# lgautier/fastq-and-furious

Hardware: AMD Instinct MI355X
Metric: GB/s FASTQ parsed (higher is better)
Workload: dtype u8; 1 GPU; single-1g; description=S-single 150 bp synthetic FASTQ, 1073741522 bytes/GPU, 3334601 records/GPU, diagnostic=False, bytes_per_gpu=1073741522, records_per_gpu=3334601, total_bytes=1073741522, total_records=3334601

## Files before the change

### fastq-and-furious_amd/csrc/ffq_rows4.h

```cpp
#pragma once
#include "ffq_chain.h"

namespace ffq {

constexpr int SB_TILES = 64;
constexpr int R4_LIST = SLOT + 8;

struct Fast4Hdr {
    long long j0;
    int32_t attempt;
    int32_t dense_seen;
    unsigned long long irr_min;
    unsigned long long term_min;
    long long n_lines;
};

struct TermInfo4 {
    int64_t pos[6];
    int32_t status;
    int32_t final_;
};

struct TileQ {
    long long kfirst;
    int32_t nrec;
    uint32_t qsum;
};

__device__ __forceinline__ long long tile_ordinal_base(const LineIndex &L, const long long *sbbase, int t, int lane)
{
    const int sb = t / SB_TILES, t0 = sb * SB_TILES;
    const uint32_t c = (t0 + lane < t) ? L.cnt[t0 + lane] : 0u;
    return sbbase[sb] + (long long)wave_sum_u32(c) + L.s;
}

__global__ __launch_bounds__(256) void k_sum64(const uint32_t *__restrict__ src, int stride, int64_t nsrc,
                                               unsigned int *__restrict__ dst, int ndst)
{
    const int b = blockIdx.x * 4 + __builtin_amdgcn_readfirstlane((int)(threadIdx.x >> 6)), lane = threadIdx.x & 63;
    if (b >= ndst) return;
    const int64_t i = (int64_t)b * 64 + lane;
    const uint32_t v = (i < nsrc) ? src[i * stride] : 0u;
    const uint32_t t = wave_sum_u32(v);
    if (lane == 0) dst[b] = t;
}

__global__ __launch_bounds__(1024) void k_sbscan(LineIndex L, int nsb, long long *__restrict__ sbbase, int64_t offset,
                                                 Fast4Hdr *hdr, const unsigned int *__restrict__ presum)
{
    __shared__ long long s_w[16];
    __shared__ uint32_t s_sum[16][64];
    const int tid = threadIdx.x, lane = tid & 63, wid = tid >> 6;
    if (wid == 15) {
        const int tq = (int)min((int64_t)max(L.ntiles - 1, 0), max((int64_t)0, (offset - L.s) >> TILE_SHIFT));
        uint32_t sink = (L.n > 0) ? (uint32_t)L.d[0] : 0u;
        if (L.ntiles > 0) sink += L.cnt[tq] + L.ent[(int64_t)tq * SLOT + lane * 4];
        if (tq + 1 < L.ntiles) sink += L.cnt[tq + 1] + L.ent[(int64_t)(tq + 1) * SLOT + (lane & 15) * 4];
        asm volatile("" ::"v"(sink));
    }
    long long carry = 0;
    if (presum) {
        for (int c0 = 0; c0 < nsb; c0 += 16 * 1024) {
            uint32_t pv[16];
#pragma unroll
            for (int k = 0; k < 16; k++) {
                const int b = c0 + k * 1024 + tid;
                pv[k] = (b < nsb) ? presum[b] : 0u;
            }
#pragma unroll
            for (int k = 0; k < 16; k++) {
                const int b = c0 + k * 1024 + tid;
                if (c0 + k * 1024 >= nsb) continue;
                const uint32_t v = pv[k];
                const uint32_t incl = wave_incl_scan(v);
                if (lane == 63) s_w[wid] = (long long)incl;
                __syncthreads();
                long long wpre = 0, tot = 0;
#pragma unroll
                for (int q = 0; q < 16; q++) {
                    const long long t = s_w[q];
                    if (q < wid) wpre += t;
                    tot += t;
                }
                if (b < nsb) sbbase[b] = carry + wpre + (long long)(incl - v);
                __syncthreads();
                carry += tot;
            }
        }
    } else
    for (int b0 = 0; b0 < nsb; b0 += 1024) {
        const int b = b0 + tid;
        uint32_t part[16];
        const int64_t tw0 = ((int64_t)(b0 + wid * 64) << 6) + lane * 4;
        if (tw0 + (15 << 8) + 4 <= L.ntiles - (63 - lane) * 4) {
            uint4 x[16];
#pragma unroll
            for (int j = 0; j < 16; j++) x[j] = *reinterpret_cast<const uint4 *>(L.cnt + tw0 + ((int64_t)j << 8));
#pragma unroll
            for (int j = 0; j < 16; j++) part[j] = x[j].x + x[j].y + x[j].z + x[j].w;
        } else {
#pragma unroll
            for (int j = 0; j < 16; j++) {
                const int64_t t = tw0 + ((int64_t)j << 8);
                uint32_t a = 0;
                for (int q = 0; q < 4; q++)
                    if (t + q < L.ntiles) a += L.cnt[t + q];
                part[j] = a;
            }
        }
#pragma unroll
        for (int j = 0; j < 16; j++) {
            uint32_t r = part[j];
            r += (uint32_t)__builtin_amdgcn_update_dpp(0, (int)r, 0x111, 0xf, 0xf, false);
            r += (uint32_t)__builtin_amdgcn_update_dpp(0, (int)r, 0x112, 0xf, 0xf, false);
            r += (uint32_t)__builtin_amdgcn_update_dpp(0, (int)r, 0x114, 0xf, 0xf, false);
            r += (uint32_t)__builtin_amdgcn_update_dpp(0, (int)r, 0x118, 0xf, 0xf, false);
            if ((lane & 15) == 15) s_sum[wid][4 * j + (lane >> 4)] = r;
        }
        __syncthreads();
        const uint32_t v = (b < nsb) ? s_sum[wid][lane] : 0u;
        const uint32_t incl = wave_incl_scan(v);
        if (lane == 63) s_w[wid] = (long long)incl;
        __syncthreads();
        long long wpre = 0, tot = 0;
#pragma unroll
        for (int q = 0; q < 16; q++) {
            const long long t = s_w[q];
            if (q < wid) wpre += t;
            tot += t;
        }
        if (b < nsb) sbbase[b] = carry + wpre + (long long)(incl - v);
        __syncthreads();
        carry += tot;
    }
    __syncthreads();
    if (tid == 0) {
        hdr->n_lines = carry;
        hdr->irr_min = ~0ull;
        hdr->term_min = ~0ull;
        hdr->attempt = 1;
        hdr->dense_seen = 0;
        hdr->j0 = -1;
        const GAcc a(L);
        H h = a.before();
        long long ord = -1;
        long long found = -1;
        int64_t P; int fl;
        int tskip = (int)min((int64_t)L.ntiles, max((int64_t)0, (offset - L.s) >> TILE_SHIFT));
        if (tskip > 0) {
            long long o = sbbase[tskip / SB_TILES] + L.s;
            for (int t = (tskip / SB_TILES) * SB_TILES; t < tskip; t++) o += L.cnt[t];
            h = H{tskip - 1, 0x7FFFFFF0};
            ord = o - 1;
        }
        bool gave_up = false;
        for (int steps = 0;; steps++) {
            if (steps > 4096) { gave_up = true; break; }
            bool ok;
            if (h.tile >= 0 && h.i == 0x7FFFFFF0) {
                int t = h.tile + 1;
                while (t < L.ntiles && L.cnt[t] == 0) t++;
                ok = t < L.ntiles;
                if (ok) { h.tile = t; h.i = 0; }
            } else ok = a.next(h);
            if (!ok) break;
            ord++;
            a.get(h, P, fl);
            if ((fl & FL_AT) && P >= offset) { found = ord; break; }
        }
        if (gave_up) hdr->attempt = 0;
        else {
            hdr->j0 = found;
            if (found >= 0) {
                H h2 = h;
                if (a.next(h2) && a.next(h2)) {
                    a.get(h2, P, fl);
                    if (!(fl & FL_PLUS)) hdr->attempt = 0;
                }
            }
        }
    }
}

constexpr uint8_t FZ_ALL = 0xFE;
template <int FUSED, bool DENSE>
__global__ __launch_bounds__(256, DENSE ? 4 : 8) void k_rows4(LineIndex L, const long long *__restrict__ sbbase, int eof,
                                               int64_t add, Fast4Hdr *hdr, TermInfo4 *__restrict__ tinfo,
                                               int64_t *__restrict__ table, int64_t table_cap,
                                               uint32_t *__restrict__ qrel, TileQ *__restrict__ tileq,
                                               int64_t *__restrict__ p4s, int64_t p4_cap,
                                               int64_t fz_stride, const uint8_t *__restrict__ fz_phase,
                                               int64_t *__restrict__ fz_qoff)
{
    __shared__ __attribute__((aligned(16))) uint16_t s_ent_all[4][R4_LIST];
    __shared__ uint32_t s_la_all[4][8];
    __shared__ __attribute__((aligned(16))) int32_t s_rows_all[4][64 * 6];
    const int wid = __builtin_amdgcn_readfirstlane((int)(threadIdx.x >> 6)), lane = threadIdx.x & 63;
    const int t = blockIdx.x * 4 + wid;
    if (t >= L.ntiles) return;
    const int attempt = hdr->attempt;
    const long long j0 = hdr->j0;
    const unsigned long long irr0 = hdr->irr_min;
    const unsigned long long term0 = hdr->term_min;
    uint16_t *s_ent = s_ent_all[wid];
    uint32_t *s_la = s_la_all[wid];
    int32_t *s_rows = s_rows_all[wid];
    const int64_t len = L.len();

    const int tn = min(t + 1, L.ntiles - 1);
    const int sb = t / SB_TILES, t0 = sb * SB_TILES;
    const uint16_t *src = L.ent + (int64_t)t * SLOT;
    const uint32_t c_raw = L.cnt[t];
    const uint2 v0 = *reinterpret_cast<const uint2 *>(src + 4 * lane);
    const uint32_t c1_raw = L.cnt[tn];
    const uint2 vla_raw = *reinterpret_cast<const uint2 *>(L.ent + (int64_t)tn * SLOT + 4 * (lane & 1));
    const uint32_t cb_raw = L.cnt[min(t0 + lane, L.ntiles - 1)];
    const long long sbb = sbbase[sb];
    constexpr bool fused = FUSED != 0, in_place = FUSED == 2;
    uint32_t fzph = 0;
    if (fused) fzph = fz_phase[t];
    asm volatile("" ::"v"(c_raw), "v"(v0.x), "v"(v0.y), "v"(c1_raw), "v"(vla_raw.x), "v"(vla_raw.y), "v"(cb_raw),
                 "v"(sbb), "s"(attempt), "s"(j0), "v"(fzph));
    const int c = (int)c_raw;
    const bool have_next = t + 1 < L.ntiles;
    const int c1 = have_next ? (int)c1_raw : 0;
    const uint2 vla = vla_raw;
    const long long ob = sbb + (long long)wave_sum_u32((t0 + lane < t) ? cb_raw : 0u) + L.s;
    if (!attempt) return;
    if (ob - j0 > 0 && ((unsigned long long)((ob - j0) >> 2) > irr0 || (unsigned long long)((ob - j0) >> 2) > (term0 >> 24))) return;
    if (c > SLOT && (!DENSE || fused)) {
        if (lane == 0 && (hdr->irr_min != 0ull || !hdr->dense_seen)) { atomicMin(&hdr->irr_min, 0ull); hdr->dense_seen = 1; }
        return;
    }
    if (fused) {
        const uint32_t want = (uint32_t)(((j0 + 3 - ob) % 4 + 4) % 4);
        const bool wrong = in_place ? (fzph != (uint32_t)FZ_ALL && fzph != want) : (c > 0 && fzph != want);
        if ((wrong || j0 != 0) && lane == 0 && hdr->irr_min != 0ull) atomicMin(&hdr->irr_min, 0ull);
    }
    const int pre = (t == 0 && L.s) ? 1 : 0;
    if (c + pre == 0 && t != 0) return;
    const int64_t tbase = ((int64_t)t << TILE_SHIFT) + L.s;
    const int64_t tb_add = tbase + add;
    const int32_t lim = (int32_t)min(len - tbase, (int64_t)0x7FFFFFF0);
    if (j0 < 0) {
        if (t == 0 && lane == 0) {
            TermInfo4 &ti = tinfo[0];
            for (int i = 0; i < 6; i++) ti.pos[i] = -1;
            ti.status = ST_HEAD_BEG; ti.final_ = 0;
            atomicMin(&hdr->term_min, 0ull);
        }
        return;
    }
    const int ntot = pre + c;
    const int nch = DENSE ? (ntot + SLOT - 1) / SLOT : 1;
    const uint16_t *dsrc = nullptr;
    if (DENSE && c > SLOT) {
        const unsigned long long at = L.ovf[t] & OVF_MASK;
        if (at + (unsigned long long)c > L.pool_cap) {
            if (lane == 0) atomicMin(&hdr->irr_min, 0ull);
            return;
        }
        dsrc = L.pool + at;
    }
    long long kfirst = -1;
    int nrec_tile = 0;
    bool tile_term_done = false;
    uint32_t qrun = 0;
    for (int ch = 0; ch < nch; ch++) {
    const int e_lo = DENSE ? ch * SLOT : 0;
    const int nown = DENSE ? min(SLOT, ntot - e_lo) : ntot;
    const bool sent0 = pre && e_lo == 0;
    const long long obl = ob - pre + e_lo;
    if (DENSE && ch > 0) wave_sync();
    if (DENSE && dsrc) {
        for (int x0 = 8 * lane; x0 < nown; x0 += 512) {
            const int ph = e_lo + x0 - pre;
            if (ph >= 0 && ph + 8 <= c) {
                typedef uint32_t u32x4u __attribute__((ext_vector_type(4), aligned(2)));
                const u32x4u v = *reinterpret_cast<const u32x4u *>(dsrc + ph);
                *reinterpret_cast<uint4 *>(s_ent + x0) = make_uint4(v.x, v.y, v.z, v.w);
            } else {
#pragma unroll
                for (int q = 0; q < 8; q++)
                    if (ph + q >= 0 && ph + q < c) s_ent[x0 + q] = dsrc[ph + q];
            }
        }
    }
    if (sent0) {
        if (lane == 0) {
            const uint8_t b0 = L.n > 0 ? L.d[0] : 0;
            const uint32_t fl = (b0 == '@') ? FL_AT : (b0 == '+') ? FL_PLUS : 0;
            s_ent[0] = (uint16_t)(fl << 14);
        }
        if (!(DENSE && dsrc)) {
            const uint32_t x[4] = {v0.x & 0xFFFFu, v0.x >> 16, v0.y & 0xFFFFu, v0.y >> 16};
#pragma unroll
            for (int i = 0; i < 4; i++)
                if (4 * lane + i < c) s_ent[1 + 4 * lane + i] = (uint16_t)x[i];
        }
    } else if (!(DENSE && dsrc)) {
        *reinterpret_cast<uint2 *>(s_ent + 4 * lane) = v0;
    }
    if (!(DENSE && dsrc))
        for (int i = 256 + lane; i < c; i += 64) {
            s_ent[pre + i] = src[i];
        }
    int nl = nown;
    bool idx_end = false;
    const bool last_ch = !DENSE || ch == nch - 1;
    bool la_simple;
    int32_t la_add = TILE;
    if (last_ch) {
        la_simple = have_next && c1 >= 5 && (c1 <= SLOT || DENSE);
        if (la_simple && (!DENSE || c1 <= SLOT)) {
            if (lane < 2) {
                const uint32_t x[4] = {vla.x & 0xFFFFu, vla.x >> 16, vla.y & 0xFFFFu, vla.y >> 16};
#pragma unroll
                for (int i = 0; i < 4; i++)
                    if (4 * lane + i < 5) {
                        s_la[4 * lane + i] = ((1u << TILE_SHIFT) + (x[i] & OFF_MASK)) | ((x[i] >> 14) << 30);
                        s_ent[nl + 4 * lane + i] = (uint16_t)x[i];
                    }
            }
            nl += 5;
        } else if (la_simple) {
            const unsigned long long at1 = L.ovf[t + 1] & OVF_MASK;
            if (at1 + 5ull <= L.pool_cap) {
                if (lane < 5) {
                    const uint32_t e = L.pool[at1 + lane];
                    s_la[lane] = ((1u << TILE_SHIFT) + (e & OFF_MASK)) | ((e >> 14) << 30);
                    s_ent[nl + lane] = (uint16_t)e;
                }
                nl += 5;
            } else la_simple = false;
        }
    } else {
        la_simple = ntot - (e_lo + nown) >= 5;
        la_add = 0;
        if (la_simple) {
            if (lane < 5) {
                const uint32_t e = dsrc[e_lo + nown - pre + lane];
                s_la[lane] = (e & OFF_MASK) | ((e >> 14) << 30);
                s_ent[nl + lane] = (uint16_t)e;
            }
            nl += 5;
        }
    }
    if (!la_simple) {
        int tt = last_ch ? t + 1 : t, pp = last_ch ? 0 : e_lo + nown - pre, got = 0;
        while (got < 5) {
            if (tt >= L.ntiles) { idx_end = true; break; }
            const int cc = (tt == t) ? c : (int)L.cnt[tt];
            if (cc > SLOT && !DENSE) break;
            if (pp >= cc) { tt++; pp = 0; if (tt - t > 60000) break; continue; }
            const uint16_t *es = L.ent + (int64_t)tt * SLOT;
            if (cc > SLOT) {
                const unsigned long long at1 = L.ovf[tt] & OVF_MASK;
                if (at1 + (unsigned long long)cc > L.pool_cap) break;
                es = L.pool + at1;
            }
            const int take = min(cc - pp, 5 - got);
            if (lane < take) {
                const uint32_t e = es[pp + lane];
                s_la[got + lane] = (((uint32_t)(tt - t) << TILE_SHIFT) + (e & OFF_MASK)) | ((e >> 14) << 30);
            }
            got += take;
            pp += take;
        }
        nl += got;
    }
    wave_sync();

    long long kfirst_ch = -1;
    int nrec_ch = 0;
    {
        long long i0 = (obl >= j0) ? ((4 - ((obl - j0) & 3)) & 3) : (j0 - obl);
        if (i0 < nown) {
            kfirst_ch = (obl + i0 - j0) >> 2;
            nrec_ch = (int)((nown - i0 + 3) >> 2);
            if (kfirst < 0) kfirst = kfirst_ch;
        }
        for (int r0 = 0; r0 < nrec_ch; r0 += 64) {
            const int r = r0 + lane;
            const bool act = r < nrec_ch;
            const int i = (int)i0 + 4 * r;
            int cls = 0;
            bool fin = false;
            int32_t f0 = 0, f1 = 0, f3 = 0, f4 = 0, f5 = 0;
            bool usual = false;
            {
                const int ic = min(i, R4_LIST - 5);
                const uint32_t e0 = s_ent[ic], e1 = s_ent[ic + 1], e2 = s_ent[ic + 2], e3 = s_ent[ic + 3],
                               e4 = s_ent[ic + 4];
                const int32_t x0 = (sent0 && ic == 0) ? -1 : (int32_t)(e0 & OFF_MASK) + ((ic >= nown) ? la_add : 0);
                const int32_t x1 = (int32_t)(e1 & OFF_MASK) + ((ic + 1 >= nown) ? la_add : 0);
                const int32_t x2 = (int32_t)(e2 & OFF_MASK) + ((ic + 2 >= nown) ? la_add : 0);
                const int32_t x3 = (int32_t)(e3 & OFF_MASK) + ((ic + 3 >= nown) ? la_add : 0);
                const int32_t x4 = (int32_t)(e4 & OFF_MASK) + ((ic + 4 >= nown) ? la_add : 0);
                const int32_t qe = x3 + x2 - x1;
                usual = act & (i + 4 < nl) & (la_simple | (i + 4 < nown))
                      & (x1 <= lim - 2)
                      & (((e2 >> 14) & FL_PLUS) != 0) & (x2 >= x1 + 2)
                      & (x2 + 2 < lim) & (x3 <= lim - 2)
                      & !((x3 - x2 - 1 > 1) & (x3 - x2 != x1 - x0))
                      & (qe + 2 < lim)
                      & (((e4 >> 14) & FL_AT) != 0) & (x4 >= qe - 1);
                f0 = x0 + 1; f1 = x1; f3 = x2; f4 = x3 + 1; f5 = qe;
                if (fused && usual && x4 != qe) atomicMin(&hdr->irr_min, (unsigned long long)(kfirst_ch + r));
            }
            if (act && !usual) {
                int64_t p0 = 0, p1 = 0, p3 = 0, p4 = 0, p5 = 0;
                int status = ST_COMPLETE;
                const long long k = kfirst_ch + r;
                const int have = nl - i;
                auto POS = [&](int q) -> int64_t {
                    const int e = i + q;
                    if (e >= nown) return tbase + (int64_t)(s_la[e - nown] & 0x3FFFFFFFu);
                    if (sent0 && e == 0) return (int64_t)0;
                    return tbase + (int64_t)(s_ent[e] & OFF_MASK);
                };
                auto FLG = [&](int q) -> uint32_t {
                    const int e = i + q;
                    return (e >= nown) ? (s_la[e - nown] >> 30) : ((uint32_t)s_ent[e] >> 14);
                };
                const int64_t P0 = POS(0);
                p0 = P0 + 1; p1 = p3 = p4 = p5 = -1;
                if (have < 2) { cls = idx_end ? 2 : 1; status = ST_HEAD_END; }
                else {
                    const int64_t P1 = POS(1);
                    if (P1 > len - 2) { cls = 2; status = ST_HEAD_END; }
                    else {
                        p1 = P1;
                        if (have < 3) { cls = idx_end ? 2 : 1; status = ST_SEQ_END; }
                        else {
                            const int64_t P2 = POS(2);
                            if (!(FLG(2) & FL_PLUS) || P2 < P1 + 2) cls = 1;
                            else {
                                p3 = P2;
                                if (P2 + 2 >= len) { cls = 2; status = ST_QUALHEAD_END; }
                                else if (have < 4) { cls = idx_end ? 2 : 1; status = ST_QUALHEAD_END; }
                                else {
                                    const int64_t P3 = POS(3);
                                    if (P3 > len - 2) { cls = 2; status = ST_QUALHEAD_END; }
                                    else if ((P3 - P2 - 1 > 1) && (P3 - P2 != P1 - P0)) { cls = 2; status = ST_INVALID; }
                                    else {
                                        p4 = P3 + 1;
                                        const int64_t qe = p4 + P2 - P1 - 1;
                                        if (qe + 2 >= len) {
                                            cls = 2; status = ST_QUAL_END;
                                            if (eof && qe < len) { p5 = qe; fin = true; }
                                        } else {
                                            p5 = qe;
                                            if (have < 5) cls = idx_end ? 3 : 1;
                                            else if (!(FLG(4) & FL_AT) || POS(4) < qe - 1) cls = 1;
                                        }
                                    }
                                }
                            }
                        }
                    }
                }
                if (fused && (cls == 0 || cls == 3 || (cls == 2 && fin)) && !(have >= 5 && POS(4) == p5)) cls = 1;
                {
                    const unsigned long long im = __ballot(cls == 1);
                    if (cls == 1 && lane == __ffsll((long long)im) - 1 &&
                        (unsigned long long)k < __hip_atomic_load(&hdr->irr_min, __ATOMIC_RELAXED, __HIP_MEMORY_SCOPE_AGENT))
                        atomicMin(&hdr->irr_min, (unsigned long long)k);
                }
                if (cls == 2 || cls == 3) {
                    const unsigned long long kk = (unsigned long long)(cls == 3 ? k + 1 : k);
                    const unsigned long long mine = (kk << 24) | (unsigned long long)(t & 0xFFFFFF);
                    if (mine < __hip_atomic_load(&hdr->term_min, __ATOMIC_RELAXED, __HIP_MEMORY_SCOPE_AGENT)) atomicMin(&hdr->term_min, mine);
                }
                f0 = (int32_t)(p0 - tbase); f1 = (int32_t)(p1 - tbase); f3 = (int32_t)(p3 - tbase);
                f4 = (int32_t)(p4 - tbase); f5 = (int32_t)(p5 - tbase);
                const unsigned long long tm = __ballot(cls == 2 || cls == 3);
                if (tm != 0ull && !tile_term_done && lane == __ffsll((long long)tm) - 1) {
                    TermInfo4 ti;
                    if (cls == 3) {
                        for (int q = 0; q < 6; q++) ti.pos[q] = -1;
                        ti.status = ST_HEAD_BEG; ti.final_ = 0;
                    } else {
                        ti.pos[0] = p0; ti.pos[1] = p1; ti.pos[2] = (p1 >= 0) ? p1 + 1 : -1;
                        ti.pos[3] = p3; ti.pos[4] = p4; ti.pos[5] = p5;
                        ti.status = status; ti.final_ = fin ? 1 : 0;
                    }
                    tinfo[t] = ti;
                }
            }
            if (__ballot(act && (cls == 2 || cls == 3)) != 0ull) tile_term_done = true;
            const bool emit = act && (cls == 0 || cls == 3 || (cls == 2 && fin));
            if (in_place) {
                if (emit && kfirst_ch + r < p4_cap) fz_qoff[kfirst_ch + r] = ((long long)t << TILE_SHIFT) + f4;
            } else if (fused) {
                const uint32_t ql = emit ? (uint32_t)(f5 - f4) : 0u;
                const uint32_t incl = wave_incl_scan(ql);
                if (emit && kfirst_ch + r < p4_cap) {
                    const int32_t x3 = f4 - 1;
                    long long q = ((long long)t + (x3 >> TILE_SHIFT)) * fz_stride;
                    if (x3 < TILE) {
                        int32_t head = 0;
                        const int e0 = (int)i0 - pre;
                        if (kfirst_ch > 0 && e0 >= 1)
                            head = (int32_t)(s_ent[e0 + pre] & OFF_MASK) - (int32_t)(s_ent[e0 - 1 + pre] & OFF_MASK) - 1;
                        q += head + (long long)(qrun + incl - ql);
                    }
                    fz_qoff[kfirst_ch + r] = q;
                }
                qrun += (uint32_t)__shfl((int)incl, 63);
            } else if (qrel) {
                const uint32_t ql = emit ? (uint32_t)(f5 - f4) : 0u;
                const uint32_t incl = wave_incl_scan(ql);
                if (act && kfirst_ch + r < p4_cap) qrel[kfirst_ch + r] = qrun + incl - ql;
                if (emit && kfirst_ch + r < p4_cap) p4s[kfirst_ch + r] = tb_add + f4;
                qrun += (uint32_t)__shfl((int)incl, 63);
            }
            int2 *mine = reinterpret_cast<int2 *>(s_rows + lane * 6);
            mine[0] = make_int2(f0, f1); mine[1] = make_int2(f1 + 1, f3); mine[2] = make_int2(f4, f5);
            wave_sync();
            const unsigned long long em = __ballot(emit);
            const int64_t rowbase = kfirst_ch + r0;
            const int2 *srcr = reinterpret_cast<const int2 *>(s_rows);
            longlong2 *dst = reinterpret_cast<longlong2 *>(table + rowbase * 6);
#pragma unroll
            for (int u = 0; u < 3; u++) {
                const int q = lane + u * 64;
                const int row = q / 3;
                if (((em >> row) & 1ull) && rowbase + row < table_cap) {
                    typedef long long i64x2 __attribute__((ext_vector_type(2)));
                    const int2 vv = srcr[q];
                    i64x2 t; t.x = tb_add + vv.x; t.y = tb_add + vv.y;
                    __builtin_nontemporal_store(t, reinterpret_cast<i64x2 *>(dst + q));
                }
            }
            wave_sync();
        }
    }
    nrec_tile += nrec_ch;
    }
    if (qrel && lane == 0 && nrec_tile > 0) tileq[t] = TileQ{kfirst, nrec_tile, qrun};
}

__global__ __launch_bounds__(1024) void k_qscan4(const unsigned int *__restrict__ sbq, int nsb,
                                                 long long *__restrict__ sbqbase)
{
    __shared__ long long s_v[1024];
    const int tid = threadIdx.x;
    long long carry = 0;
    for (int b0 = 0; b0 < nsb; b0 += 1024) {
        const int b = b0 + tid;
        const long long v = (b < nsb) ? (long long)sbq[b] : 0;
        s_v[tid] = v;
        __syncthreads();
        for (int d = 1; d < 1024; d <<= 1) {
            long long x = 0;
            if (tid >= d) x = s_v[tid - d];
            __syncthreads();
            s_v[tid] += x;
            __syncthreads();
        }
        if (b < nsb) sbqbase[b] = carry + s_v[tid] - v;
        const long long tot = s_v[1023];
        __syncthreads();
        carry += tot;
    }
}

__global__ __launch_bounds__(256) void k_qfix4(int ntiles, const Fast4Hdr *__restrict__ hdr,
                                               const TileQ *__restrict__ tileq,
                                               const long long *__restrict__ sbqbase,
                                               const uint32_t *__restrict__ qrel, int64_t *__restrict__ qoff,
                                               int64_t table_cap, int64_t *__restrict__ qdir, int64_t qdir_cap)
{
    const int wid = __builtin_amdgcn_readfirstlane((int)(threadIdx.x >> 6)), lane = threadIdx.x & 63;
    const int t = (blockIdx.x * 4 + wid) * 2;
    if (t >= ntiles) return;
    const int attempt = hdr->attempt;
    const int t0 = (t / SB_TILES) * SB_TILES;
    const TileQ me0 = tileq[t];
    TileQ me1 = tileq[min(t + 1, ntiles - 1)];
    const uint32_t bq = tileq[min(t0 + lane, ntiles - 1)].qsum;
    const long long sbb = sbqbase[t / SB_TILES];
    asm volatile("" ::"v"(me0.kfirst), "v"(me0.nrec), "v"(me0.qsum), "v"(me1.kfirst), "v"(me1.nrec), "v"(me1.qsum),
                 "v"(bq), "v"(sbb), "s"(attempt));
    if (!attempt) return;
    if (t + 1 >= ntiles) me1.nrec = 0;
    const int64_t base0 = sbb + (int64_t)wave_sum_u32((t0 + lane < t) ? bq : 0u);
    const int64_t base1 = base0 + (int64_t)(me0.nrec > 0 ? me0.qsum : 0u);
    const int64_t i0 = me0.kfirst + lane, i1 = me1.kfirst + lane;
    const bool a0 = lane < me0.nrec && i0 < table_cap, a1 = lane < me1.nrec && i1 < table_cap;
    const int64_t l0 = a0 ? (int64_t)qrel[i0] : 0, l1 = a1 ? (int64_t)qrel[i1] : 0;
    asm volatile("" ::"v"(l0), "v"(l1));
    auto fix = [&](const TileQ &me, int64_t base, int r0, int64_t loc, bool act) {
        const int r = r0 + lane;
        const int64_t idx = me.kfirst + r;
        int64_t nxt = ((int64_t)__shfl((int)(loc >> 32), lane + 1) << 32) | (uint32_t)__shfl((int)(uint32_t)loc, lane + 1);
        if (r + 1 >= me.nrec) nxt = me.qsum;
        else if (lane == 63) nxt = (idx + 1 < table_cap) ? (int64_t)qrel[idx + 1] : (int64_t)me.qsum;
        if (act) {
            qoff[idx] = base + loc;
            qdir_mark(qdir, qdir_cap, base + loc, nxt - loc, idx);
        }
    };
    auto rest = [&](const TileQ &me, int64_t base) {
        for (int r0 = 64; r0 < me.nrec; r0 += 64) {
            const int64_t idx = me.kfirst + r0 + lane;
            const bool act = r0 + lane < me.nrec && idx < table_cap;
            fix(me, base, r0, act ? (int64_t)qrel[idx] : 0, act);
        }
    };
    if (me0.nrec > 0) fix(me0, base0, 0, l0, a0);
    if (me1.nrec > 0) fix(me1, base1, 0, l1, a1);
    if (me0.nrec > 64) rest(me0, base0);
    if (me1.nrec > 64) rest(me1, base1);
}

__global__ void k_qtotal4(DevRes *res, const int64_t *__restrict__ table, int64_t table_cap,
                          int64_t *__restrict__ qoff, Pub pb)
{
    if (threadIdx.x != 0 || blockIdx.x != 0) return;
    if (res->fallback) { publish(pb, res); return; }
    const int64_t n = res->n_records;
    int64_t tot = 0;
    if (n > 0 && n <= table_cap) tot = qoff[n - 1] + (table[(n - 1) * 6 + 5] - table[(n - 1) * 6 + 4]);
    res->n_qual_bytes = tot;
    if (n <= table_cap) qoff[n] = tot;
    publish(pb, res);
}

__global__ void k_finalize4(LineIndex L, Fast4Hdr *hdr, const TermInfo4 *__restrict__ tinfo, int eof,
                            int64_t offset, int64_t add, const int64_t *__restrict__ table, int64_t table_cap,
                            DevRes *res, Pub pb, const uint32_t *__restrict__ fz_bad = nullptr)
{
    if (threadIdx.x != 0 || blockIdx.x != 0) return;
    res->n_lines = hdr->n_lines;
    res->n_qual_bytes = 0;
    res->term_group = -1;
    res->has_final = 0;
    const unsigned long long tm = hdr->term_min, im = hdr->irr_min;
    const unsigned long long tk = tm >> 24;
    res->fused_bad = fz_bad ? (int32_t)*fz_bad : 0;
    res->fast4_dense = hdr->dense_seen;
    if (!hdr->attempt || tm == ~0ull || (im != ~0ull && im <= tk) || (fz_bad && *fz_bad)) { res->fallback = 1; res->fast4_hint = 0; publish(pb, res); return; }
    res->fallback = 0;
    res->fast4_hint = 1;
    const int tt = (int)(tm & 0xFFFFFF);
    const TermInfo4 ti = tinfo[tt];
    const int status = ti.status;
    res->last_status = status;
    for (int i = 0; i < 6; i++) res->last_pos[i] = (ti.pos[i] >= 0) ? ti.pos[i] + add : -1;
    const long long ncomplete = (long long)tk;
    res->n_records = ncomplete + (ti.final_ ? 1 : 0);
    res->has_final = ti.final_ ? 1 : 0;
    int end;
    if (ti.final_) end = 0;
    else if (status == ST_HEAD_BEG) end = eof ? 0 : 1;
    else if (eof) end = (status == ST_QUAL_END) ? 2 : (status == ST_INVALID) ? 4 : 3;
    else end = (status == ST_INVALID) ? 4 : 1;
    res->end_state = end;
    if (ncomplete > 0 && ncomplete <= table_cap) res->end_offset = table[(ncomplete - 1) * 6 + 5] - add - 1;
    else res->end_offset = offset;
    publish(pb, res);
}

}
```

Measured before the change: 4974 GB/s.

## Resolve first record start with a wave-parallel window search in sbscan

```diff
diff --git a/fastq-and-furious_amd/csrc/ffq_rows4.h b/fastq-and-furious_amd/csrc/ffq_rows4.h
--- a/fastq-and-furious_amd/csrc/ffq_rows4.h
+++ b/fastq-and-furious_amd/csrc/ffq_rows4.h
@@ -5,6 +5,7 @@
 
 constexpr int SB_TILES = 64;
 constexpr int R4_LIST = SLOT + 8;
+constexpr int SB_WIN = 1 + 256 + 64;
 
 struct Fast4Hdr {
     long long j0;
@@ -50,13 +51,62 @@
 {
     __shared__ long long s_w[16];
     __shared__ uint32_t s_sum[16][64];
+    __shared__ uint32_t s_win[SB_WIN];
+    __shared__ long long s_sbT;
+    __shared__ int32_t s_found[4];
     const int tid = threadIdx.x, lane = tid & 63, wid = tid >> 6;
+    const int tw = (int)min((int64_t)L.ntiles, max((int64_t)0, (offset - L.s) >> TILE_SHIFT));
     if (wid == 15) {
-        const int tq = (int)min((int64_t)max(L.ntiles - 1, 0), max((int64_t)0, (offset - L.s) >> TILE_SHIFT));
-        uint32_t sink = (L.n > 0) ? (uint32_t)L.d[0] : 0u;
-        if (L.ntiles > 0) sink += L.cnt[tq] + L.ent[(int64_t)tq * SLOT + lane * 4];
-        if (tq + 1 < L.ntiles) sink += L.cnt[tq + 1] + L.ent[(int64_t)(tq + 1) * SLOT + (lane & 15) * 4];
-        asm volatile("" ::"v"(sink));
+        const int tq = min(max(L.ntiles - 1, 0), tw);
+        const int tn = min(tq + 1, max(L.ntiles - 1, 0));
+        const int t0 = (tq / SB_TILES) * SB_TILES;
+        uint32_t b0 = 0, cq = 0, cn = 0, cb = 0;
+        uint2 vq = make_uint2(0u, 0u), vn = make_uint2(0u, 0u);
+        if (L.n > 0) b0 = (uint32_t)L.d[0];
+        if (L.ntiles > 0) {
+            cq = L.cnt[tq];
+            cn = L.cnt[tn];
+            cb = L.cnt[min(t0 + lane, L.ntiles - 1)];
+            vq = *reinterpret_cast<const uint2 *>(L.ent + (int64_t)tq * SLOT + lane * 4);
+            vn = *reinterpret_cast<const uint2 *>(L.ent + (int64_t)tn * SLOT + (lane & 15) * 4);
+        }
+        asm volatile("" ::"v"(b0), "v"(cq), "v"(cn), "v"(cb), "v"(vq.x), "v"(vq.y), "v"(vn.x), "v"(vn.y));
+        const uint32_t insum = wave_sum_u32((t0 + lane < tq) ? cb : 0u);
+        const bool usable = L.ntiles > 0 && tw < L.ntiles && L.ready >= L.ntiles && cq >= 1u && cq <= (uint32_t)SLOT;
+        const int pre = (tq == 0 && L.s) ? 1 : 0;
+        const int n0 = (int)min(cq, 256u);
+        const int n1 = (cq <= 256u && tq + 1 < L.ntiles && cn <= (uint32_t)SLOT) ? (int)min(cn, 64u) : 0;
+        const int nwin = pre + n0 + n1;
+        if (lane == 0 && pre) s_win[0] = ((b0 == '@') ? (uint32_t)FL_AT : (b0 == '+') ? (uint32_t)FL_PLUS : 0u) << 30;
+        const uint32_t xq[4] = {vq.x & 0xFFFFu, vq.x >> 16, vq.y & 0xFFFFu, vq.y >> 16};
+        const uint32_t xn[4] = {vn.x & 0xFFFFu, vn.x >> 16, vn.y & 0xFFFFu, vn.y >> 16};
+#pragma unroll
+        for (int i = 0; i < 4; i++) {
+            const int j = 4 * lane + i;
+            if (j < n0) s_win[pre + j] = (xq[i] & OFF_MASK) | ((xq[i] >> 14) << 30);
+            if (lane < 16 && j < n1) s_win[pre + n0 + j] = ((xn[i] & OFF_MASK) + (uint32_t)TILE) | ((xn[i] >> 14) << 30);
+        }
+        wave_sync();
+        const int64_t need = offset - (((int64_t)tq << TILE_SHIFT) + L.s);
+        int w = -1;
+        if (usable)
+            for (int r0 = 0; r0 < nwin && w < 0; r0 += 64) {
+                const int i = r0 + lane;
+                bool ok = false;
+                if (i < nwin) {
+                    const uint32_t e = s_win[i];
+                    ok = ((e >> 30) & (uint32_t)FL_AT) && ((pre && i == 0) ? offset <= 0 : (int64_t)(e & 0x3FFFFFFFu) >= need);
+                }
+                const unsigned long long m = __ballot(ok);
+                if (m) w = r0 + __ffsll((long long)m) - 1;
+            }
+        if (lane == 0) {
+            const bool decided = w >= 0 && w + 2 < nwin;
+            s_found[0] = decided ? 1 : 0;
+            s_found[1] = w;
+            s_found[2] = (decided && !((s_win[w + 2] >> 30) & (uint32_t)FL_PLUS)) ? 0 : 1;
+            s_found[3] = (int32_t)insum;
+        }
     }
     long long carry = 0;
     if (presum) {
@@ -83,6 +133,7 @@
                     tot += t;
                 }
                 if (b < nsb) sbbase[b] = carry + wpre + (long long)(incl - v);
+                if (b == tw / SB_TILES) s_sbT = carry + wpre + (long long)(incl - v);
                 __syncthreads();
                 carry += tot;
             }
@@ -130,6 +181,7 @@
             tot += t;
         }
         if (b < nsb) sbbase[b] = carry + wpre + (long long)(incl - v);
+        if (b == tw / SB_TILES) s_sbT = carry + wpre + (long long)(incl - v);
         __syncthreads();
         carry += tot;
     }
@@ -141,6 +193,11 @@
         hdr->attempt = 1;
         hdr->dense_seen = 0;
         hdr->j0 = -1;
+        if (s_found[0]) {
+            hdr->j0 = (tw == 0 ? 0ll : s_sbT + (long long)L.s + (long long)s_found[3]) + (long long)s_found[1];
+            hdr->attempt = s_found[2];
+            return;
+        }
         const GAcc a(L);
         H h = a.before();
         long long ord = -1;
```

New measurement: 4985 GB/s, median of 6. Within noise of the previous version (+0.2%).
